# Aleph-Alpha/magma

Measured on NVIDIA H100. Metric: image-caption samples/sec (fwd+bwd), higher is better.
Workload: dtype bf16

## Files before the change

### include/magma_b200.h

```cpp
#ifndef MAGMA_B200_H_
#define MAGMA_B200_H_

#include <stddef.h>
#include <stdint.h>

#ifdef __cplusplus
extern "C" {
#endif

#define MB200_VERSION 100

enum {
  MB200_OK = 0,
  MB200_E_SHAPE = -1,
  MB200_E_DTYPE = -2,
  MB200_E_ALIGN = -3,
  MB200_E_ARCH = -4,
  MB200_E_CUDA = -5,
  MB200_E_NCCL = -6,
  MB200_E_ARG = -7
};

enum { MB200_BF16 = 0, MB200_F32 = 1 };

// ... 15 lines not shown
int mb200_check_device(void);
int mb200_set_gemm_sm_limit(int n_sms);
int mb200_set_optimizer_grid(int n_blocks);
long long mb200_launch_count(void);
int mb200_prof_enable(int on);
int mb200_prof_read(double* gemm_ms, double* gemm_flops, double* gemm_bytes, long long* gemm_launches);

typedef struct {
  const void* ptr;
  int64_t ld;
  int64_t bs0, bs1;
  int32_t mn_major;
  int32_t static_data;
} mb200_operand;

typedef struct {
  int32_t M, N, K;
  int32_t nb0, nb1;
  int32_t c_dtype;
  mb200_operand A, B;
  void* C;
  int64_t ldc, c_bs0, c_bs1;
  float alpha;
  int32_t act;
  int32_t dact;
  int32_t accumulate;
  const void* bias;
  void* aux_out;
  const void* aux_in;
  const void* res1;
  const void* res2;
  int64_t ld_res;
  int32_t force_bn;
  int32_t rope_mode;
  const void* rope_tab;
  int32_t rope_S, rope_hd, rope_rot, rope_ncols;
  void* splitk_ws;
  int64_t splitk_ws_bytes;
} mb200_gemm_args;

int mb200_gemm(const mb200_gemm_args* args, void* stream);


int mb200_layernorm_fwd(const void* x, int64_t ldx, const void* gamma, const void* beta, void* y, int64_t ldy,
                        float* mean, float* rstd, int32_t rows, int32_t d, float eps, void* stream);
int mb200_layernorm_bwd(const void* dy, int64_t lddy, const void* x, int64_t ldx, const void* gamma,
                        const float* mean, const float* rstd, const void* res, int64_t ldres, void* dx, int64_t lddx,
                        int32_t rows, int32_t d, void* stream);
int mb200_layernorm_param_grad(const void* dy, int64_t lddy, const void* x, int64_t ldx, const float* mean,
                               const float* rstd, float* dgamma, float* dbeta, int32_t rows, int32_t d,
                               int32_t accumulate, void* stream);
int mb200_layernorm_param_grad_rows(const void* dy, int64_t lddy, const void* x, int64_t ldx, const float* mean,
                                    const float* rstd, float* dgamma, float* dbeta, int32_t rows, int32_t d,
                                    int32_t accumulate, void* stream);
int mb200_rope(void* qkv, int64_t ld, int32_t rows, int32_t S, int32_t H, int32_t hd, int32_t rot, int32_t pos0,
               int32_t inverse, void* stream);
int mb200_rope_table(float* tab, int32_t S, int32_t rot, int32_t pos0, void* stream);
int mb200_softmax_fwd(const float* s, int64_t lds, int64_t s_bs, void* p, int64_t ldp, int64_t p_bs, int32_t nz,
                      int32_t Sq, int32_t Sk, float scale, int32_t causal, int32_t koff, void* stream);
int mb200_softmax_bwd(const float* dp, int64_t lddp, int64_t dp_bs, const void* p, int64_t ldp, int64_t p_bs,
                      void* ds, int64_t ldds, int64_t ds_bs, int32_t nz, int32_t Sq, int32_t Sk, float scale,
                      void* stream);
int mb200_build_labels(const int64_t* captions, int64_t ldc, int64_t* labels, int32_t B, int32_t S, int32_t L,
                       int64_t eos, void* stream);
int mb200_embed_assemble(const int64_t* captions, int64_t ldc, const void* wte, const void* prefix, int32_t L,
                         void* x, int32_t B, int32_t S, int32_t d, int32_t vocab, void* stream);
// ... 201 lines not shown
```

### magma_b200/_lib.py

```python
import ctypes
import os

_HERE = os.path.dirname(os.path.abspath(__file__))
LIB_PATH = os.path.join(_HERE, "lib", "libmagma_b200.so")

_lib = None


class MB200Error(RuntimeError):
    pass


class Operand(ctypes.Structure):
    _fields_ = [
        ("ptr", ctypes.c_void_p),
        ("ld", ctypes.c_int64),
        ("bs0", ctypes.c_int64),
        ("bs1", ctypes.c_int64),
        ("mn_major", ctypes.c_int32),
        ("static_data", ctypes.c_int32),
    ]


class GemmArgs(ctypes.Structure):
    _fields_ = [
        ("M", ctypes.c_int32),
        ("N", ctypes.c_int32),
        ("K", ctypes.c_int32),
        ("nb0", ctypes.c_int32),
        ("nb1", ctypes.c_int32),
        ("c_dtype", ctypes.c_int32),
        ("A", Operand),
        ("B", Operand),
        ("C", ctypes.c_void_p),
        ("ldc", ctypes.c_int64),
        ("c_bs0", ctypes.c_int64),
        ("c_bs1", ctypes.c_int64),
        ("alpha", ctypes.c_float),
        ("act", ctypes.c_int32),
        ("dact", ctypes.c_int32),
        ("accumulate", ctypes.c_int32),
        ("bias", ctypes.c_void_p),
        ("aux_out", ctypes.c_void_p),
        ("aux_in", ctypes.c_void_p),
        ("res1", ctypes.c_void_p),
        ("res2", ctypes.c_void_p),
        ("ld_res", ctypes.c_int64),
        ("force_bn", ctypes.c_int32),
        ("rope_mode", ctypes.c_int32),
        ("rope_tab", ctypes.c_void_p),
        ("rope_S", ctypes.c_int32),
        ("rope_hd", ctypes.c_int32),
        ("rope_rot", ctypes.c_int32),
        ("rope_ncols", ctypes.c_int32),
        ("splitk_ws", ctypes.c_void_p),
        ("splitk_ws_bytes", ctypes.c_int64),
    ]


def lib():
    global _lib
    if _lib is None:
        if not os.path.exists(LIB_PATH):
            raise MB200Error(
                f"{LIB_PATH} not found: build it with `python -m magma_b200.build` "
                "(magma_b200 has no CPU / eager fallback)"
            )
        L = ctypes.CDLL(LIB_PATH)
        L.mb200_last_error.restype = ctypes.c_char_p
        L.mb200_version.restype = ctypes.c_int
        _setup_signatures(L)
        _lib = L
    return _lib


def check(rc):
    if rc != 0:
        raise MB200Error(f"magma_b200 error {rc}: {lib().mb200_last_error().decode()}")


class VitLayerC(ctypes.Structure):
# ... 105 lines not shown
```

### magma_b200/csrc/gemm.cu

```cuda
#include <mutex>
#include <stdlib.h>

#include "gemm_common.cuh"

namespace mb200 {

template <bool kOn>
struct EpiMaps {
  CUtensorMap m[3];
};
template <>
struct EpiMaps<false> {};

template <int BN, bool A_MN, bool B_MN, bool EPI_TMA>
__global__ void __launch_bounds__(kThreads, 1)
gemm_wgmma_kernel(const __grid_constant__ CUtensorMap tmA, const __grid_constant__ CUtensorMap tmB,
                  const __grid_constant__ EpiMaps<EPI_TMA> tmE, const __grid_constant__ GemmKernelParams p) {
  using C_ = Cfg<BN>;
  constexpr int kStages = C_::kStages;

  extern __shared__ uint8_t smem_raw[];
  uint8_t* smem = reinterpret_cast<uint8_t*>((reinterpret_cast<uintptr_t>(smem_raw) + 1023) & ~uintptr_t(1023));
  uint8_t* smem_a = smem;
  uint8_t* smem_b = smem + kStages * C_::kABytes;
  float* epi_stage = reinterpret_cast<float*>(smem + kStages * C_::kStageBytes);
  uint64_t* full_bar = reinterpret_cast<uint64_t*>(smem + kStages * C_::kStageBytes + kEpiBytes);
  uint64_t* empty_bar = full_bar + kStages;
  const EpiRing ring{smem_a, smem_b, full_bar, empty_bar};

  const int wg = threadIdx.x >> 7;
  const int num_kb = (p.K + BK - 1) / BK;
  const int items = p.total_tiles * p.split_k;

  pdl_trigger();
  if (threadIdx.x == 0) {
    tma_prefetch_desc(&tmA);
    tma_prefetch_desc(&tmB);
    if constexpr (EPI_TMA) {
#pragma unroll 1
      for (int i = 0; i < p.epi_in; ++i) tma_prefetch_desc(&tmE.m[i]);
    }
    for (int s = 0; s < kStages; ++s) {
      mbar_init(&full_bar[s], 1);
      mbar_init(&empty_bar[s], 2);
    }
    mbar_fence_init();
  }
  __syncthreads();
  pdl_wait();

  if (wg == 0) {
    setmaxnreg_dec<40>();
    if (threadIdx.x == 0) {
      int stage = 0;
      uint32_t phase = 0;
// ... 47 lines not shown
    for (int w = blockIdx.x; w < items; w += gridDim.x) {
      const int t = w / p.split_k, ks = w - t * p.split_k;
      const int kb0 = ks * p.kb_per_split, kb1 = min(num_kb, kb0 + p.kb_per_split);
      const int tpb = p.tiles_m * p.tiles_n;
      const int z = t / tpb;
      const int r = t - z * tpb;
      const int m_blk = r % p.tiles_m;
      const int n_blk = r / p.tiles_m;
      const int z0 = z % p.nb0, z1 = z / p.nb0;
      int prev = -1;
      for (int kb = kb0; kb < kb1; ++kb) {
        mbar_wait(&full_bar[stage], phase);
        const uint32_t sa = smem_u32(smem_a + stage * C_::kABytes) + a_off;
        const uint32_t sb = smem_u32(smem_b + stage * C_::kBBytes);
        wgmma_fence();
#pragma unroll
        for (int k = 0; k < BK / WG_K; ++k) {
          const uint64_t da = make_smem_desc(sa + k * a_kadv, 0u, 1024);
          const uint64_t db = make_smem_desc(sb + k * b_kadv, b_lbo, 1024);
          wgmma_bf16<BN, A_MN ? 1 : 0, B_MN ? 1 : 0>(acc, da, db, (kb > kb0 || k > 0) ? 1u : 0u);
        }
        wgmma_commit();
        wgmma_wait<1>();
        if (prev >= 0 && leader) mbar_arrive(&empty_bar[prev]);
        prev = stage;
        if (++stage == kStages) {
          stage = 0;
          phase ^= 1;
        }
      }
      wgmma_wait<0>();
      if (prev >= 0 && leader) mbar_arrive(&empty_bar[prev]);
      const long long boff = (long long)z0 * p.c_bs0 + (long long)z1 * p.c_bs1;
      epi_tile<BN, EPI_TMA>(p, acc, epi_stage + cw * 64 * kEpiCols, 1 + cw, boff, m_blk * BM + cw * 64, n_blk * BN, ks, ring,
                   stage, phase);
    }
  }
}

__global__ void splitk_finalize_kernel(const GemmKernelParams p) {
  pdl_trigger();
  pdl_wait();
  const int ncol4 = (p.N + 3) >> 2;
  const long long total = (long long)p.M * ncol4;
  for (long long i = blockIdx.x * (long long)blockDim.x + threadIdx.x; i < total; i += (long long)gridDim.x * blockDim.x) {
    const int row = (int)(i / ncol4);
    const int col = (int)(i - (long long)row * ncol4) * 4;
    float v[4] = {0.f, 0.f, 0.f, 0.f};
    for (int ks = 0; ks < p.split_k; ++ks) {
      const float4 w4 = *reinterpret_cast<const float4*>(p.splitk_ws + ((long long)ks * p.M + row) * p.ld_ws + col);
      v[0] += w4.x;
      v[1] += w4.y;
      v[2] += w4.z;
      v[3] += w4.w;
    }
    EpiIn in;
    if (p.bias) ld_bf16x4(p.bias + col, min(4, p.N - col), in.bias);
    epi_load_inputs(p, 0, row, col, in);
    epi_store4(p, 0, row, col, v, in);
  }
}

typedef CUresult (*PFN_encodeTiled)(CUtensorMap*, CUtensorMapDataType, cuuint32_t, void*, const cuuint64_t*,
                                    const cuuint64_t*, const cuuint32_t*, const cuuint32_t*, CUtensorMapInterleave,
                                    CUtensorMapSwizzle, CUtensorMapL2promotion, CUtensorMapFloatOOBfill);

static PFN_encodeTiled get_encode_fn() {
  static PFN_encodeTiled fn = nullptr;
  static std::once_flag once;
  std::call_once(once, [] {
    void* p = nullptr;
    cudaDriverEntryPointQueryResult qres;
    if (cudaGetDriverEntryPoint("cuTensorMapEncodeTiled", &p, cudaEnableDefault, &qres) == cudaSuccess &&
        qres == cudaDriverEntryPointSuccess)
      fn = reinterpret_cast<PFN_encodeTiled>(p);
  });
  return fn;
}

int make_operand_map(CUtensorMap* out, const mb200_operand& op, int rows, int K, int nb0, int nb1,
                            int box_rows) {
  PFN_encodeTiled enc = get_encode_fn();
  MB_REQUIRE(enc != nullptr, MB200_E_CUDA, "cuTensorMapEncodeTiled entry point unavailable");
  MB_REQUIRE((reinterpret_cast<uintptr_t>(op.ptr) & 15) == 0, MB200_E_ALIGN, "gemm operand pointer not 16B aligned");
  MB_REQUIRE(op.ld % 8 == 0, MB200_E_ALIGN, "gemm operand ld (%lld) must be a multiple of 8 elements",
             (long long)op.ld);
  MB_REQUIRE((nb0 == 1 || op.bs0 % 8 == 0) && (nb1 == 1 || op.bs1 % 8 == 0), MB200_E_ALIGN,
             "gemm operand batch strides must be multiples of 8 elements");
  cuuint64_t dims[4];
  cuuint64_t strides[3];
  cuuint32_t box[4];
  cuuint32_t estr[4] = {1, 1, 1, 1};
  if (!op.mn_major) {
    dims[0] = (cuuint64_t)K;
    dims[1] = (cuuint64_t)rows;
    box[0] = BK;
    box[1] = (cuuint32_t)box_rows;
  } else {
    dims[0] = (cuuint64_t)rows;
    dims[1] = (cuuint64_t)K;
    box[0] = 64;
    box[1] = BK;
  }
  dims[2] = (cuuint64_t)nb0;
  dims[3] = (cuuint64_t)nb1;
  box[2] = 1;
  box[3] = 1;
  strides[0] = (cuuint64_t)op.ld * 2;
  strides[1] = (cuuint64_t)(nb0 > 1 ? op.bs0 : op.ld) * 2;
  strides[2] = (cuuint64_t)(nb1 > 1 ? op.bs1 : op.ld) * 2;
  CUresult r = enc(out, CU_TENSOR_MAP_DATA_TYPE_BFLOAT16, 4, const_cast<void*>(op.ptr), dims, strides, box, estr,
                   CU_TENSOR_MAP_INTERLEAVE_NONE, CU_TENSOR_MAP_SWIZZLE_128B, CU_TENSOR_MAP_L2_PROMOTION_L2_256B,
                   CU_TENSOR_MAP_FLOAT_OOB_FILL_NONE);
  MB_REQUIRE(r == CUDA_SUCCESS, MB200_E_CUDA,
             "cuTensorMapEncodeTiled failed (%d): dims=(%llu,%llu,%llu,%llu) strides=(%llu,%llu,%llu) box=(%u,%u)",
             (int)r, (unsigned long long)dims[0], (unsigned long long)dims[1], (unsigned long long)dims[2],
             (unsigned long long)dims[3], (unsigned long long)strides[0], (unsigned long long)strides[1],
             (unsigned long long)strides[2], box[0], box[1]);
  return 0;
}

template <int BN, bool A_MN, bool B_MN, bool EPI_TMA>
static int launch_gemm(const CUtensorMap& tmA, const CUtensorMap& tmB, const EpiMaps<true>& tmE,
                       const GemmKernelParams& kp, cudaStream_t stream) {
  auto kern = gemm_wgmma_kernel<BN, A_MN, B_MN, EPI_TMA>;
  static bool attr_set = false;
  if (!attr_set) {
    MB_CUDA(cudaFuncSetAttribute(kern, cudaFuncAttributeMaxDynamicSharedMemorySize, Cfg<BN>::kSmemBytes));
    attr_set = true;
  }
  const long long items = (long long)kp.total_tiles * kp.split_k;
  int grid = items < gemm_sms() ? (int)items : gemm_sms();
  {
    const double nb = (double)kp.total_tiles / ((double)kp.tiles_m * kp.tiles_n);
    const double flops = 2.0 * kp.M * (double)kp.N * kp.K * nb;
    const double bytes = nb * (2.0 * ((double)kp.M * kp.K + (double)kp.N * kp.K) + (kp.c_f32 ? 4.0 : 2.0) * kp.M * kp.N);
    GemmProfScope prof(stream, flops, bytes);
    if constexpr (EPI_TMA)
      MB_CUDA(launch_pdl(kern, dim3(grid), dim3(kThreads), Cfg<BN>::kSmemBytes, stream, tmA, tmB, tmE, kp));
    else
      MB_CUDA(launch_pdl(kern, dim3(grid), dim3(kThreads), Cfg<BN>::kSmemBytes, stream, tmA, tmB, EpiMaps<false>{}, kp));
  }
  count_launch();
  MB_CUDA(cudaGetLastError());
  return 0;
}

template <int BN, bool EPI_TMA>
static int dispatch_major(bool a_mn, bool b_mn, const CUtensorMap& tmA, const CUtensorMap& tmB,
                          const EpiMaps<true>& tmE, const GemmKernelParams& kp, cudaStream_t s) {
  if (!a_mn && !b_mn) return launch_gemm<BN, false, false, EPI_TMA>(tmA, tmB, tmE, kp, s);
  if (!a_mn && b_mn) return launch_gemm<BN, false, true, EPI_TMA>(tmA, tmB, tmE, kp, s);
  if (a_mn && !b_mn) return launch_gemm<BN, true, false, EPI_TMA>(tmA, tmB, tmE, kp, s);
  return launch_gemm<BN, true, true, EPI_TMA>(tmA, tmB, tmE, kp, s);
}

static int dispatch_bn(int bn, bool a_mn, bool b_mn, const CUtensorMap& tmA, const CUtensorMap& tmB,
                       const EpiMaps<true>& tmE, const GemmKernelParams& kp, cudaStream_t s) {
  const bool epi = kp.epi_in != 0;
  switch (bn) {
    case 64:
      return epi ? dispatch_major<64, true>(a_mn, b_mn, tmA, tmB, tmE, kp, s)
                 : dispatch_major<64, false>(a_mn, b_mn, tmA, tmB, tmE, kp, s);
    case 128:
      return epi ? dispatch_major<128, true>(a_mn, b_mn, tmA, tmB, tmE, kp, s)
                 : dispatch_major<128, false>(a_mn, b_mn, tmA, tmB, tmE, kp, s);
    default:
      return epi ? dispatch_major<256, true>(a_mn, b_mn, tmA, tmB, tmE, kp, s)
                 : dispatch_major<256, false>(a_mn, b_mn, tmA, tmB, tmE, kp, s);
  }
}

static int make_epi_maps(EpiMaps<true>* maps, GemmKernelParams* kp, const mb200_gemm_args* a) {
  const void* ptr[3];
  long long ld[3];
  int n = 0;
  if (a->dact) {
    ptr[n] = a->aux_in;
    ld[n++] = a->ldc;
  }
  if (a->res1) {
    ptr[n] = a->res1;
    ld[n++] = a->ld_res;
  }
  if (a->res2) {
    ptr[n] = a->res2;
    ld[n++] = a->ld_res;
  }
  bool ok = (a->nb0 == 1 || a->c_bs0 % 8 == 0) && (a->nb1 == 1 || a->c_bs1 % 8 == 0);
  for (int i = 0; i < n; ++i) ok = ok && (reinterpret_cast<uintptr_t>(ptr[i]) & 15) == 0 && ld[i] % 8 == 0;
  if (n == 0 || !ok) return 0;
  for (int i = 0; i < n; ++i) {
    mb200_operand op;
    memset(&op, 0, sizeof(op));
    op.ptr = ptr[i];
    op.ld = ld[i];
    op.bs0 = a->c_bs0;
    op.bs1 = a->c_bs1;
    const int rc = make_operand_map(&maps->m[i], op, a->M, a->N, a->nb0, a->nb1, BM);
    if (rc) return rc;
  }
  kp->epi_in = n;
  return 0;
// ... 145 lines not shown
    }
    const long long ld_ws = (a->N + 3) / 4 * 4;
    while (split > 1 && (size_t)split * a->M * ld_ws * sizeof(float) > (size_t)a->splitk_ws_bytes) --split;
    if (split > 1) {
      const int kb_per = (num_kb + split - 1) / split;
      split = (num_kb + kb_per - 1) / kb_per;
      bn = bn_s;
      rc = make_operand_map(&tmB, a->B, a->N, a->K, a->nb0, a->nb1, bn);
      if (rc) return rc;
      kp.tiles_n = tiles;
      kp.total_tiles = tiles_m * tiles;
      kp.split_k = split;
      kp.kb_per_split = kb_per;
      kp.splitk_ws = reinterpret_cast<float*>(a->splitk_ws);
      kp.ld_ws = ld_ws;
      GemmKernelParams kg = kp;
      kg.epi_kind = EK_SPLITK;
      rc = dispatch_bn(bn, amn, bmn, tmA, tmB, tmE, kg, stream);
      if (rc) return rc;
      const long long n4 = (long long)a->M * ((a->N + 3) / 4);
      const int fgrid = (int)((n4 + 255) / 256 > 2048 ? 2048 : (n4 + 255) / 256);
      kp.alpha = 1.f;
      MB_CUDA(launch_pdl(splitk_finalize_kernel, dim3(fgrid), dim3(256), 0, stream, kp));
      count_launch();
      return 0;
    }
  }
  rc = make_operand_map(&tmB, a->B, a->N, a->K, a->nb0, a->nb1, bn);
  if (rc) return rc;
  kp.tiles_n = (a->N + bn - 1) / bn;
  kp.total_tiles = tiles_m * kp.tiles_n * a->nb0 * a->nb1;
  rc = make_epi_maps(&tmE, &kp, a);
  if (rc) return rc;
  return dispatch_bn(bn, amn, bmn, tmA, tmB, tmE, kp, stream);
}

}

extern "C" int mb200_gemm(const mb200_gemm_args* args, void* stream) {
  return mb200::gemm_impl(args, reinterpret_cast<cudaStream_t>(stream));
}
```

### magma_b200/csrc/gemm_common.cuh

```cuda
#pragma once
#include "common.cuh"

namespace mb200 {

static constexpr int BM = 128;
static constexpr int BK = 64;
static constexpr int WG_K = 16;
static constexpr int kThreads = 384;
static constexpr int kEpiCols = 64;
static constexpr int kEpiBytes = BM * kEpiCols * 4;
static constexpr int kEpiBoxBytes = BM * kEpiCols * 2;
static constexpr int kSmemBudget = 192 * 1024;

template <int BN>
struct Cfg {
  static constexpr int kABytes = BM * BK * 2;
  static constexpr int kBBytes = BN * BK * 2;
  static constexpr int kStageBytes = kABytes + kBBytes;
  static constexpr int kStagesRaw = kSmemBudget / kStageBytes;
  static constexpr int kStages = kStagesRaw > 8 ? 8 : kStagesRaw;
  static constexpr int kSmemBytes = kStages * kStageBytes + kEpiBytes + 1024  + 256 ;
  static_assert(kSmemBytes <= 227 * 1024, "GEMM shared memory exceeds the sm_90 per-block limit");
  static constexpr int kEpiBoxesPerStage = 1 + kBBytes / kEpiBoxBytes;
  static_assert(kABytes == kEpiBoxBytes && kEpiBoxesPerStage * kEpiBoxBytes <= kStageBytes, "epilogue box layout");
  static_assert(3 * (BN / kEpiCols) <= kStages * kEpiBoxesPerStage, "epilogue inputs exceed the operand ring");
};

struct GemmKernelParams {
  int M, N, K;
  int nb0;
  int tiles_m, tiles_n, total_tiles;
  void* C;
  long long ldc, c_bs0, c_bs1;
  float alpha;
  int act, dact, accumulate;
  const bf16* bias;
  bf16* aux_out;
  const bf16* aux_in;
  const bf16* res1;
  const bf16* res2;
  long long ld_res;
  int epi_in;
  const float2* rope_tab;
  int rope_mode;
  int rope_S, rope_hd, rope_rot, rope_ncols;
  int epi_kind;
  int c_f32;
  int split_k, kb_per_split;
  float* splitk_ws;
  long long ld_ws;
};

__device__ __forceinline__ float2 bf16x2_to_f32(uint32_t u) {
  return __bfloat1622float2(*reinterpret_cast<const __nv_bfloat162*>(&u));
}
__device__ __forceinline__ uint32_t f32x2_to_bf16(float a, float b) {
  __nv_bfloat162 h = __floats2bfloat162_rn(a, b);
  return *reinterpret_cast<uint32_t*>(&h);
}

__device__ __forceinline__ void ld_bf16x4(const bf16* src, int n, float (&v)[4]) {
  if (n == 4 && (reinterpret_cast<uintptr_t>(src) & 7) == 0) {
    uint32_t u0, u1;
    asm volatile("ld.global.nc.v2.u32 {%0, %1}, [%2];" : "=r"(u0), "=r"(u1) : "l"(src));
    const float2 a = bf16x2_to_f32(u0), b = bf16x2_to_f32(u1);
    v[0] = a.x;
    v[1] = a.y;
    v[2] = b.x;
    v[3] = b.y;
  } else {
#pragma unroll
    for (int e = 0; e < 4; ++e) v[e] = e < n ? __bfloat162float(src[e]) : 0.f;
  }
}
__device__ __forceinline__ void st_bf16x4(bf16* dst, int n, const float (&v)[4]) {
  if (n == 4 && (reinterpret_cast<uintptr_t>(dst) & 7) == 0) {
    *reinterpret_cast<uint2*>(dst) = make_uint2(f32x2_to_bf16(v[0], v[1]), f32x2_to_bf16(v[2], v[3]));
  } else {
#pragma unroll
    for (int e = 0; e < 4; ++e)
      if (e < n) dst[e] = __float2bfloat16(v[e]);
  }
}

__device__ __forceinline__ void named_bar_sync(int id, int nthreads) {
  asm volatile("bar.sync %0, %1;" ::"r"(id), "r"(nthreads) : "memory");
}

enum { EK_GENERIC = 0, EK_SPLITK };

struct EpiIn {
  float bias[4], aux[4], res1[4], res2[4];
};

__device__ __forceinline__ void epi_load_inputs(const GemmKernelParams& p, long long boff, int row, int col,
                                                EpiIn& in) {
  const int n = min(4, p.N - col);
  if (p.dact) ld_bf16x4(p.aux_in + boff + (long long)row * p.ldc + col, n, in.aux);
  const long long roff = boff + (long long)row * p.ld_res + col;
  if (p.res1) ld_bf16x4(p.res1 + roff, n, in.res1);
  if (p.res2) ld_bf16x4(p.res2 + roff, n, in.res2);
}

__device__ __forceinline__ void ld_smem_bf16x4(const uint8_t* src, float (&v)[4]) {
  const uint2 u = *reinterpret_cast<const uint2*>(src);
  const float2 a = bf16x2_to_f32(u.x), b = bf16x2_to_f32(u.y);
  v[0] = a.x;
  v[1] = a.y;
  v[2] = b.x;
  v[3] = b.y;
}

__device__ __forceinline__ void epi_store4(const GemmKernelParams& p, long long boff, int row, int col, float (&v)[4],
                                           const EpiIn& in) {
  const int n = min(4, p.N - col);
  if (p.bias) {
#pragma unroll
    for (int e = 0; e < 4; ++e) v[e] += in.bias[e];
  }
  if (p.rope_mode != 0 && col < p.rope_ncols) {
    const int dim = col % p.rope_hd;
    if (dim < p.rope_rot) {
      const float2* tp = p.rope_tab + (long long)(row % p.rope_S) * (p.rope_rot >> 1) + (dim >> 1);
      const float2 cs0 = __ldg(tp), cs1 = __ldg(tp + 1);
      const float sg = p.rope_mode > 0 ? 1.f : -1.f;
      const float a0 = v[0], a1 = v[1], a2 = v[2], a3 = v[3];
      v[0] = a0 * cs0.x - a1 * cs0.y * sg;
      v[1] = a1 * cs0.x + a0 * cs0.y * sg;
      v[2] = a2 * cs1.x - a3 * cs1.y * sg;
      v[3] = a3 * cs1.x + a2 * cs1.y * sg;
    }
  }
  const long long coff = boff + (long long)row * p.ldc + col;
  if (p.aux_out) st_bf16x4(p.aux_out + coff, n, v);
#pragma unroll
  for (int e = 0; e < 4; ++e) {
    if (p.act == MB200_ACT_GELU_NEW) v[e] = gelu_new_f(v[e]);
    else if (p.act == MB200_ACT_QUICK_GELU) v[e] = quick_gelu_f(v[e]);
    else if (p.act == MB200_ACT_RELU) v[e] = fmaxf(v[e], 0.f);
  }
  if (p.dact) {
#pragma unroll
    for (int e = 0; e < 4; ++e)
      v[e] = p.dact == MB200_DACT_GELU_NEW ? v[e] * gelu_new_grad_f(in.aux[e]) : (in.aux[e] > 0.f ? v[e] : 0.f);
  }
  if (p.res1) {
#pragma unroll
    for (int e = 0; e < 4; ++e) v[e] += in.res1[e];
  }
  if (p.res2) {
#pragma unroll
    for (int e = 0; e < 4; ++e) v[e] += in.res2[e];
  }
  if (p.act == MB200_ACT_RELU_POST) {
#pragma unroll
    for (int e = 0; e < 4; ++e) v[e] = fmaxf(v[e], 0.f);
  }
  if (p.c_f32) {
    float* dst = reinterpret_cast<float*>(p.C) + coff;
    if (n == 4) {
      float4 o = make_float4(v[0], v[1], v[2], v[3]);
      if (p.accumulate) {
        const float4 old = *reinterpret_cast<const float4*>(dst);
        o.x += old.x;
        o.y += old.y;
        o.z += old.z;
        o.w += old.w;
      }
      *reinterpret_cast<float4*>(dst) = o;
    } else {
#pragma unroll
      for (int e = 0; e < 4; ++e)
        if (e < n) dst[e] = p.accumulate ? dst[e] + v[e] : v[e];
    }
  } else {
    st_bf16x4(reinterpret_cast<bf16*>(p.C) + coff, n, v);
  }
}


struct EpiRing {
  uint8_t* a;
  uint8_t* b;
  uint64_t* full;
  uint64_t* empty;
};

template <int BN>
__device__ __forceinline__ int epi_chunks(const GemmKernelParams& p, int col0) {
  return min(BN / kEpiCols, (p.N - col0 + kEpiCols - 1) / kEpiCols);
}

template <int BN>
__device__ __forceinline__ uint8_t* epi_box(const EpiRing& ring, int s, int k) {
  return k == 0 ? ring.a + s * Cfg<BN>::kABytes : ring.b + s * Cfg<BN>::kBBytes + (k - 1) * kEpiBoxBytes;
}

template <int BN, bool EPI_TMA>
__device__ __forceinline__ void epi_tile(const GemmKernelParams& p, const float (&acc)[BN / 2], float* stage,
                                         int bar_id, long long boff, int row0, int col0, int ks, const EpiRing& ring,
                                         int& ring_stage, uint32_t& ring_phase) {
  constexpr int kStages = Cfg<BN>::kStages, kBps = Cfg<BN>::kEpiBoxesPerStage;
  const int wt = threadIdx.x & 127;
  const int fr = (wt >> 5) * 16 + ((wt & 31) >> 2);
  const int fq = wt & 3;
  const int pr = wt >> 4, pc = wt & 15;
  const int nch = epi_chunks<BN>(p, col0);
  const int nin = EPI_TMA ? p.epi_in : 0;
  int bs = ring_stage, bk = 0, rs = ring_stage;
  uint32_t bph = ring_phase;
  auto next_box = [&]() {
    if (bk == 0) mbar_wait(&ring.full[bs], bph);
    const uint8_t* box = epi_box<BN>(ring, bs, bk);
    if (++bk == kBps) {
      bk = 0;
      if (++bs == kStages) {
        bs = 0;
        bph ^= 1;
      }
    }
    return box;
  };
  const int box_off = ((row0 % BM) + pr) * 128 + (((pc >> 1) ^ pr) << 4) + ((pc & 1) << 3);
#pragma unroll 1
  for (int ch = 0; ch < nch; ++ch) {
#pragma unroll
    for (int c = 0; c < BN / kEpiCols; ++c) {
      if (c != ch) continue;
#pragma unroll
      for (int jj = 0; jj < 8; ++jj) {
        const int j = c * 8 + jj;
#pragma unroll
        for (int h = 0; h < 2; ++h) {
          const int r = fr + 8 * h;
          const int q = (2 * jj + (fq >> 1)) ^ ((r & 3) << 1);
          *reinterpret_cast<float2*>(stage + r * kEpiCols + q * 4 + 2 * (fq & 1)) =
              make_float2(acc[4 * j + 2 * h], acc[4 * j + 2 * h + 1]);
        }
      }
    }
    named_bar_sync(bar_id, 128);
    const int col = col0 + ch * kEpiCols + pc * 4;
    const uint8_t *src_aux = nullptr, *src_res1 = nullptr, *src_res2 = nullptr;
    if (nin) {
      if (p.dact) src_aux = next_box() + box_off;
      if (p.res1) src_res1 = next_box() + box_off;
      if (p.res2) src_res2 = next_box() + box_off;
    }
    EpiIn in;
    if (p.bias && col < p.N) ld_bf16x4(p.bias + col, min(4, p.N - col), in.bias);
#pragma unroll 1
    for (int i = 0; i < 64 / 8; ++i) {
      const int r = pr + 8 * i;
      const int row = row0 + r;
      if (row >= p.M || col >= p.N) continue;
      const float4 s = *reinterpret_cast<const float4*>(stage + r * kEpiCols + ((pc ^ ((r & 3) << 1)) * 4));
      float v[4] = {s.x * p.alpha, s.y * p.alpha, s.z * p.alpha, s.w * p.alpha};
      if (p.epi_kind == EK_SPLITK) {
        *reinterpret_cast<float4*>(p.splitk_ws + ((long long)ks * p.M + row) * p.ld_ws + col) =
            make_float4(v[0], v[1], v[2], v[3]);
        continue;
      }
      if (nin) {
        if (p.dact) ld_smem_bf16x4(src_aux + i * 1024, in.aux);
        if (p.res1) ld_smem_bf16x4(src_res1 + i * 1024, in.res1);
        if (p.res2) ld_smem_bf16x4(src_res2 + i * 1024, in.res2);
      } else {
        epi_load_inputs(p, boff, row, col, in);
      }
      epi_store4(p, boff, row, col, v, in);
    }
    named_bar_sync(bar_id, 128);
    if (nin) {
      if (ch + 1 == nch && bk != 0) {
        bk = 0;
        if (++bs == kStages) {
          bs = 0;
          bph ^= 1;
        }
      }
#pragma unroll 1
      for (; rs != bs; rs = rs + 1 == kStages ? 0 : rs + 1)
        if (wt == 0) mbar_arrive(&ring.empty[rs]);
    }
  }
  ring_stage = bs;
  ring_phase = bph;
}

template <int BN>
__device__ __forceinline__ void epi_queue_inputs(const GemmKernelParams& p, const CUtensorMap* maps,
                                                 const EpiRing& ring, int& stage, uint32_t& phase, int m0, int col0,
                                                 int z0, int z1) {
  constexpr int kStages = Cfg<BN>::kStages, kBps = Cfg<BN>::kEpiBoxesPerStage;
  const int nbox = p.epi_in * epi_chunks<BN>(p, col0);
  int col = col0, i = 0;
#pragma unroll 1
  for (int b0 = 0; b0 < nbox; b0 += kBps) {
    const int nb = min(kBps, nbox - b0);
    mbar_wait(&ring.empty[stage], phase ^ 1);
    mbar_expect_tx(&ring.full[stage], (uint32_t)(nb * kEpiBoxBytes));
#pragma unroll 1
    for (int k = 0; k < nb; ++k) {
// ... 17 lines not shown
```

### magma_b200/ops.py

```python
import ctypes

import torch

from . import _lib
from ._lib import GemmArgs, check, lib

ACT_NONE, ACT_GELU_NEW, ACT_QUICK_GELU, ACT_RELU, ACT_RELU_POST = 0, 1, 2, 3, 4
DACT_NONE, DACT_GELU_NEW, DACT_RELU = 0, 1, 3


def _stream():
    return ctypes.c_void_p(torch.cuda.current_stream().cuda_stream)


def _ptr(t):
    return ctypes.c_void_p(t.data_ptr()) if t is not None else None


def _mat_meta(t, name):
    if t.dim() < 2 or t.dim() > 4:
        raise ValueError(f"{name}: expected 2-4 dims, got {t.dim()}")
    if t.stride(-1) != 1 and t.shape[-1] != 1:
        raise ValueError(f"{name}: innermost stride must be 1, got {t.stride()}")
    rows, cols = t.shape[-2], t.shape[-1]
    ld = t.stride(-2) if rows > 1 else max(cols, t.stride(-2))
    nb0 = t.shape[-3] if t.dim() >= 3 else 1
    bs0 = t.stride(-3) if t.dim() >= 3 else 0
    nb1 = t.shape[-4] if t.dim() >= 4 else 1
    bs1 = t.stride(-4) if t.dim() >= 4 else 0
    return rows, cols, ld, nb0, nb1, bs0, bs1


def gemm(
    A,
    B,
    out=None,
    *,
    a_mn=False,
    b_mn=False,
    out_dtype=torch.bfloat16,
    alpha=1.0,
    bias=None,
    act=ACT_NONE,
    aux_out=None,
    aux_in=None,
    dact=DACT_NONE,
    res1=None,
    res2=None,
    accumulate=False,
    force_bn=0,
    rope_tab=None,
    rope_mode=0,
    rope_S=0,
    rope_hd=0,
    rope_rot=0,
    rope_ncols=0,
    splitk_ws=None,
    b_static=False,
):
    if A.dtype != torch.bfloat16 or B.dtype != torch.bfloat16:
        raise TypeError("gemm operands must be bf16")
    ra, ca, lda, anb0, anb1, abs0, abs1 = _mat_meta(A, "A")
    rb, cb, ldb, bnb0, bnb1, bbs0, bbs1 = _mat_meta(B, "B")
    M, K = (ca, ra) if a_mn else (ra, ca)
    N, Kb = (cb, rb) if b_mn else (rb, cb)
    if K != Kb:
        raise ValueError(f"gemm K mismatch: {K} vs {Kb}")
    nb0, nb1 = max(anb0, bnb0), max(anb1, bnb1)
    if (anb0, anb1) != (nb0, nb1) or (bnb0, bnb1) != (nb0, nb1):
        raise ValueError("gemm: A and B must have identical batch dims")
    if out is None:
        shape = ([nb1] if A.dim() >= 4 else []) + ([nb0] if A.dim() >= 3 else []) + [M, N]
        out = torch.empty(shape, dtype=out_dtype, device=A.device)
    rc_, cc, ldc, cnb0, cnb1, cbs0, cbs1 = _mat_meta(out, "out")
    if (rc_, cc) != (M, N) or (cnb0, cnb1) != (nb0, nb1):
        raise ValueError(f"gemm: out shape {tuple(out.shape)} does not match M={M} N={N} batch=({nb1},{nb0})")
    g = GemmArgs()
    g.M, g.N, g.K, g.nb0, g.nb1 = M, N, K, nb0, nb1
    g.c_dtype = 1 if out.dtype == torch.float32 else 0
    if out.dtype not in (torch.float32, torch.bfloat16):
        raise TypeError("gemm out must be bf16 or f32")
    g.A.ptr, g.A.ld, g.A.bs0, g.A.bs1, g.A.mn_major = A.data_ptr(), lda, abs0, abs1, int(a_mn)
    g.B.ptr, g.B.ld, g.B.bs0, g.B.bs1, g.B.mn_major = B.data_ptr(), ldb, bbs0, bbs1, int(b_mn)
    g.B.static_data = int(bool(b_static))
    g.C, g.ldc, g.c_bs0, g.c_bs1 = out.data_ptr(), ldc, cbs0, cbs1
    g.alpha, g.act, g.dact, g.accumulate = float(alpha), int(act), int(dact), int(bool(accumulate))
    for name, t in (("bias", bias), ("aux_out", aux_out), ("aux_in", aux_in), ("res1", res1), ("res2", res2)):
        if t is not None:
            if t.dtype != torch.bfloat16:
                raise TypeError(f"gemm {name} must be bf16")
            setattr(g, name, t.data_ptr())
    if bias is not None and (tuple(bias.shape) != (N,) or (N > 1 and bias.stride(0) != 1)):
        raise ValueError(f"gemm bias must be a contiguous [N={N}] vector, got shape {tuple(bias.shape)}")
    for name, t in (("aux_out", aux_out), ("aux_in", aux_in), ("res1", res1), ("res2", res2)):
        if t is not None and tuple(t.shape) != tuple(out.shape):
            raise ValueError(f"gemm {name} shape {tuple(t.shape)} must equal out's {tuple(out.shape)}")
    for name, t in (("aux_out", aux_out), ("aux_in", aux_in)):
        if t is not None and _mat_meta(t, name)[2:] != (ldc, cnb0, cnb1, cbs0, cbs1):
            raise ValueError(f"gemm {name} must share out's strides")
    ld_res = 0
    for name, t in (("res1", res1), ("res2", res2)):
        if t is not None:
            m = _mat_meta(t, name)
            if (cnb0 > 1 and m[5] != cbs0) or (cnb1 > 1 and m[6] != cbs1):
                raise ValueError(f"gemm {name} must share out's batch strides (its row stride may differ)")
            if ld_res and m[2] != ld_res:
                raise ValueError("res1/res2 must share a row stride")
            ld_res = m[2]
    g.ld_res = ld_res
    g.force_bn = force_bn
    if rope_tab is not None and rope_mode:
        g.rope_tab, g.rope_mode = rope_tab.data_ptr(), int(rope_mode)
        g.rope_S, g.rope_hd, g.rope_rot, g.rope_ncols = int(rope_S), int(rope_hd), int(rope_rot), int(rope_ncols)
    if splitk_ws is not None:
        g.splitk_ws, g.splitk_ws_bytes = splitk_ws.data_ptr(), splitk_ws.numel() * splitk_ws.element_size()
    check(lib().mb200_gemm(ctypes.byref(g), _stream()))
    return out


def _rows(t):
    d = t.shape[-1]
    if t.dim() == 1:
        return 1, d, d
    t2 = t.reshape(-1, d) if t.is_contiguous() else None
    if t2 is not None:
        return t2.shape[0], d, d
    if t.dim() == 2:
        return t.shape[0], d, t.stride(0)
    raise ValueError("non-contiguous >2-D tensor: pass a 2-D view with an explicit row stride")


def layernorm_fwd(x, gamma, beta, eps=1e-5, save_stats=True, out=None):
    rows, d, ldx = _rows(x)
    y = torch.empty(x.shape, dtype=torch.bfloat16, device=x.device) if out is None else out
    mean = torch.empty(rows, dtype=torch.float32, device=x.device) if save_stats else None
    rstd = torch.empty(rows, dtype=torch.float32, device=x.device) if save_stats else None
    check(lib().mb200_layernorm_fwd(_ptr(x), ctypes.c_int64(ldx), _ptr(gamma), _ptr(beta), _ptr(y),
                                    ctypes.c_int64(_rows(y)[2]), _ptr(mean), _ptr(rstd), rows, d,
                                    ctypes.c_float(eps), _stream()))
    return y, mean, rstd


def layernorm_bwd(dy, x, gamma, mean, rstd, res=None, out=None):
# ... 413 lines not shown
```

Measured before the change: 136.7.

## Specialize GEMM epilogue at compile time for common fusion forms

Adds compile-time epilogue variants (EpiForm) for a set of common fused-epilogue combinations: bias, GELU, aux output, residuals, dGELU, RoPE and f32 output. A host-side dispatcher picks the matching specialized kernel when BN is 256 and the alignment checks pass. Specialized forms drop runtime branches, process 8 rows per unrolled batch and use unconditional vector loads and stores. This is meant to cut epilogue instruction overhead and raise memory-level parallelism, at the cost of more kernel instantiations, longer compile time and higher register pressure.

After: 155.5 (median of 6 runs). 13.7% higher.

```diff
diff --git a/include/magma_b200.h b/include/magma_b200.h
--- a/include/magma_b200.h
+++ b/include/magma_b200.h
@@ -71,6 +71,7 @@
   const void* res2;
   int64_t ld_res;
   int32_t force_bn;
+  int32_t generic_epilogue;
   int32_t rope_mode;
   const void* rope_tab;
   int32_t rope_S, rope_hd, rope_rot, rope_ncols;
diff --git a/magma_b200/_lib.py b/magma_b200/_lib.py
--- a/magma_b200/_lib.py
+++ b/magma_b200/_lib.py
@@ -47,6 +47,7 @@
         ("res2", ctypes.c_void_p),
         ("ld_res", ctypes.c_int64),
         ("force_bn", ctypes.c_int32),
+        ("generic_epilogue", ctypes.c_int32),
         ("rope_mode", ctypes.c_int32),
         ("rope_tab", ctypes.c_void_p),
         ("rope_S", ctypes.c_int32),
diff --git a/magma_b200/csrc/gemm.cu b/magma_b200/csrc/gemm.cu
--- a/magma_b200/csrc/gemm.cu
+++ b/magma_b200/csrc/gemm.cu
@@ -12,7 +12,7 @@
 template <>
 struct EpiMaps<false> {};
 
-template <int BN, bool A_MN, bool B_MN, bool EPI_TMA>
+template <int BN, bool A_MN, bool B_MN, bool EPI_TMA, uint32_t FORM = EF_RUNTIME>
 __global__ void __launch_bounds__(kThreads, 1)
 gemm_wgmma_kernel(const __grid_constant__ CUtensorMap tmA, const __grid_constant__ CUtensorMap tmB,
                   const __grid_constant__ EpiMaps<EPI_TMA> tmE, const __grid_constant__ GemmKernelParams p) {
@@ -20,7 +20,7 @@
   constexpr int kStages = C_::kStages;
 
   extern __shared__ uint8_t smem_raw[];
-  uint8_t* smem = reinterpret_cast<uint8_t*>((reinterpret_cast<uintptr_t>(smem_raw) + 1023) & ~uintptr_t(1023));
+  uint8_t* smem = smem_raw + ((1024u - (smem_u32(smem_raw) & 1023u)) & 1023u);
   uint8_t* smem_a = smem;
   uint8_t* smem_b = smem + kStages * C_::kABytes;
   float* epi_stage = reinterpret_cast<float*>(smem + kStages * C_::kStageBytes);
@@ -134,8 +134,8 @@
       wgmma_wait<0>();
       if (prev >= 0 && leader) mbar_arrive(&empty_bar[prev]);
       const long long boff = (long long)z0 * p.c_bs0 + (long long)z1 * p.c_bs1;
-      epi_tile<BN, EPI_TMA>(p, acc, epi_stage + cw * 64 * kEpiCols, 1 + cw, boff, m_blk * BM + cw * 64, n_blk * BN, ks, ring,
-                   stage, phase);
+      epi_tile<BN, EPI_TMA, EpiForm<FORM>>(p, acc, epi_stage + cw * 64 * kEpiCols, 1 + cw, boff, m_blk * BM + cw * 64,
+                                           n_blk * BN, ks, ring, stage, phase);
     }
   }
 }
@@ -156,10 +156,12 @@
       v[2] += w4.z;
       v[3] += w4.w;
     }
+    using Form = EpiForm<EF_RUNTIME>;
+    float bias[4];
     EpiIn in;
-    if (p.bias) ld_bf16x4(p.bias + col, min(4, p.N - col), in.bias);
-    epi_load_inputs(p, 0, row, col, in);
-    epi_store4(p, 0, row, col, v, in);
+    if (p.bias) ld_bf16x4(p.bias + col, min(4, p.N - col), bias);
+    epi_load_inputs<Form>(p, 0, row, col, in);
+    epi_store4<Form>(p, 0, row, col, v, bias, in);
   }
 }
 
@@ -222,10 +224,10 @@
   return 0;
 }
 
-template <int BN, bool A_MN, bool B_MN, bool EPI_TMA>
+template <int BN, bool A_MN, bool B_MN, bool EPI_TMA, uint32_t FORM = EF_RUNTIME>
 static int launch_gemm(const CUtensorMap& tmA, const CUtensorMap& tmB, const EpiMaps<true>& tmE,
                        const GemmKernelParams& kp, cudaStream_t stream) {
-  auto kern = gemm_wgmma_kernel<BN, A_MN, B_MN, EPI_TMA>;
+  auto kern = gemm_wgmma_kernel<BN, A_MN, B_MN, EPI_TMA, FORM>;
   static bool attr_set = false;
   if (!attr_set) {
     MB_CUDA(cudaFuncSetAttribute(kern, cudaFuncAttributeMaxDynamicSharedMemorySize, Cfg<BN>::kSmemBytes));
@@ -271,6 +273,41 @@
       return epi ? dispatch_major<256, true>(a_mn, b_mn, tmA, tmB, tmE, kp, s)
                  : dispatch_major<256, false>(a_mn, b_mn, tmA, tmB, tmE, kp, s);
   }
+}
+
+template <uint32_t F, bool A_MN, bool B_MN>
+static bool launch_form(uint32_t form, bool a_mn, bool b_mn, const CUtensorMap& tmA, const CUtensorMap& tmB,
+                        const EpiMaps<true>& tmE, const GemmKernelParams& kp, cudaStream_t s, int* rc) {
+  if (form != F || a_mn != A_MN || b_mn != B_MN) return false;
+  *rc = launch_gemm<256, A_MN, B_MN, EpiForm<F>::kInputs != 0, F>(tmA, tmB, tmE, kp, s);
+  return true;
+}
+static bool dispatch_form(uint32_t form, bool a_mn, bool b_mn, const CUtensorMap& tmA, const CUtensorMap& tmB,
+                          const EpiMaps<true>& tmE, const GemmKernelParams& kp, cudaStream_t s, int* rc) {
+#define MB_FORM(F, A_MN, B_MN) launch_form<(F), A_MN, B_MN>(form, a_mn, b_mn, tmA, tmB, tmE, kp, s, rc)
+  return MB_FORM(EF_ROPE, false, false) ||
+         MB_FORM(EF_RES1, false, false) ||
+         MB_FORM(EF_BIAS | EF_GELU | EF_AUX_OUT, false, false) ||
+         MB_FORM(EF_BIAS, false, false) ||
+         MB_FORM(EF_BIAS | EF_RES1 | EF_RES2, false, false) ||
+         MB_FORM(EF_DGELU, false, true) ||
+         MB_FORM(0u, false, true) ||
+         MB_FORM(EF_RES1, false, true) ||
+         MB_FORM(EF_F32, true, true);
+#undef MB_FORM
+}
+
+static uint32_t epi_form(const mb200_gemm_args* a, const GemmKernelParams& kp, int bn) {
+  if (a->generic_epilogue || bn != 256) return EF_RUNTIME;
+  if ((a->act != MB200_ACT_NONE && a->act != MB200_ACT_GELU_NEW) ||
+      (a->dact != MB200_DACT_NONE && a->dact != MB200_DACT_GELU_NEW))
+    return EF_RUNTIME;
+  if (((reinterpret_cast<uintptr_t>(a->bias) | reinterpret_cast<uintptr_t>(a->aux_out)) & 7) != 0) return EF_RUNTIME;
+  const uint32_t f = (a->bias ? EF_BIAS : 0u) | (kp.rope_mode ? EF_ROPE : 0u) | (a->aux_out ? EF_AUX_OUT : 0u) |
+                     (a->act ? EF_GELU : 0u) | (a->dact ? EF_DGELU : 0u) | (a->res1 ? EF_RES1 : 0u) |
+                     (a->res2 ? EF_RES2 : 0u) | (kp.c_f32 ? EF_F32 : 0u);
+  const int inputs = (a->dact != 0) + (a->res1 != nullptr) + (a->res2 != nullptr);
+  return kp.epi_in == inputs ? f : EF_RUNTIME;
 }
 
 static int make_epi_maps(EpiMaps<true>* maps, GemmKernelParams* kp, const mb200_gemm_args* a) {
@@ -482,6 +519,7 @@
   kp.total_tiles = tiles_m * kp.tiles_n * a->nb0 * a->nb1;
   rc = make_epi_maps(&tmE, &kp, a);
   if (rc) return rc;
+  if (dispatch_form(epi_form(a, kp, bn), amn, bmn, tmA, tmB, tmE, kp, stream, &rc)) return rc;
   return dispatch_bn(bn, amn, bmn, tmA, tmB, tmE, kp, stream);
 }
 
diff --git a/magma_b200/csrc/gemm_common.cuh b/magma_b200/csrc/gemm_common.cuh
--- a/magma_b200/csrc/gemm_common.cuh
+++ b/magma_b200/csrc/gemm_common.cuh
@@ -1,4 +1,6 @@
 #pragma once
+#include <type_traits>
+
 #include "common.cuh"
 
 namespace mb200 {
@@ -59,8 +61,9 @@
   return *reinterpret_cast<uint32_t*>(&h);
 }
 
+template <bool kVec = false>
 __device__ __forceinline__ void ld_bf16x4(const bf16* src, int n, float (&v)[4]) {
-  if (n == 4 && (reinterpret_cast<uintptr_t>(src) & 7) == 0) {
+  if (kVec || (n == 4 && (reinterpret_cast<uintptr_t>(src) & 7) == 0)) {
     uint32_t u0, u1;
     asm volatile("ld.global.nc.v2.u32 {%0, %1}, [%2];" : "=r"(u0), "=r"(u1) : "l"(src));
     const float2 a = bf16x2_to_f32(u0), b = bf16x2_to_f32(u1);
@@ -73,8 +76,9 @@
     for (int e = 0; e < 4; ++e) v[e] = e < n ? __bfloat162float(src[e]) : 0.f;
   }
 }
+template <bool kVec = false>
 __device__ __forceinline__ void st_bf16x4(bf16* dst, int n, const float (&v)[4]) {
-  if (n == 4 && (reinterpret_cast<uintptr_t>(dst) & 7) == 0) {
+  if (kVec || (n == 4 && (reinterpret_cast<uintptr_t>(dst) & 7) == 0)) {
     *reinterpret_cast<uint2*>(dst) = make_uint2(f32x2_to_bf16(v[0], v[1]), f32x2_to_bf16(v[2], v[3]));
   } else {
 #pragma unroll
@@ -89,17 +93,54 @@
 
 enum { EK_GENERIC = 0, EK_SPLITK };
 
+enum : uint32_t {
+  EF_BIAS = 1,
+  EF_ROPE = 2,
+  EF_AUX_OUT = 4,
+  EF_GELU = 8,
+  EF_DGELU = 16,
+  EF_RES1 = 32,
+  EF_RES2 = 64,
+  EF_F32 = 128,
+  EF_RUNTIME = 1u << 31
+};
+
+template <uint32_t F>
+struct EpiForm {
+  static constexpr bool kRuntime = F == EF_RUNTIME;
+  static constexpr int kInputs = kRuntime ? 0 : ((F & EF_DGELU) != 0) + ((F & EF_RES1) != 0) + ((F & EF_RES2) != 0);
+  static constexpr int kRows = kRuntime ? 1 : 8;
+  using P = GemmKernelParams;
+  static __device__ __forceinline__ bool bias(const P& p) { return kRuntime ? p.bias != nullptr : (F & EF_BIAS) != 0; }
+  static __device__ __forceinline__ bool rope(const P& p) { return kRuntime ? p.rope_mode != 0 : (F & EF_ROPE) != 0; }
+  static __device__ __forceinline__ bool aux_out(const P& p) {
+    return kRuntime ? p.aux_out != nullptr : (F & EF_AUX_OUT) != 0;
+  }
+  static __device__ __forceinline__ int act(const P& p) {
+    return kRuntime ? p.act : (F & EF_GELU) ? MB200_ACT_GELU_NEW : MB200_ACT_NONE;
+  }
+  static __device__ __forceinline__ int dact(const P& p) {
+    return kRuntime ? p.dact : (F & EF_DGELU) ? MB200_DACT_GELU_NEW : MB200_DACT_NONE;
+  }
+  static __device__ __forceinline__ bool res1(const P& p) { return kRuntime ? p.res1 != nullptr : (F & EF_RES1) != 0; }
+  static __device__ __forceinline__ bool res2(const P& p) { return kRuntime ? p.res2 != nullptr : (F & EF_RES2) != 0; }
+  static __device__ __forceinline__ bool c_f32(const P& p) { return kRuntime ? p.c_f32 != 0 : (F & EF_F32) != 0; }
+  static __device__ __forceinline__ bool accumulate(const P& p) { return (kRuntime || (F & EF_F32)) && p.accumulate; }
+  static __device__ __forceinline__ bool splitk(const P& p) { return kRuntime && p.epi_kind == EK_SPLITK; }
+};
+
 struct EpiIn {
-  float bias[4], aux[4], res1[4], res2[4];
-};
-
+  float aux[4], res1[4], res2[4];
+};
+
+template <class Form>
 __device__ __forceinline__ void epi_load_inputs(const GemmKernelParams& p, long long boff, int row, int col,
                                                 EpiIn& in) {
   const int n = min(4, p.N - col);
-  if (p.dact) ld_bf16x4(p.aux_in + boff + (long long)row * p.ldc + col, n, in.aux);
+  if (Form::dact(p)) ld_bf16x4(p.aux_in + boff + (long long)row * p.ldc + col, n, in.aux);
   const long long roff = boff + (long long)row * p.ld_res + col;
-  if (p.res1) ld_bf16x4(p.res1 + roff, n, in.res1);
-  if (p.res2) ld_bf16x4(p.res2 + roff, n, in.res2);
+  if (Form::res1(p)) ld_bf16x4(p.res1 + roff, n, in.res1);
+  if (Form::res2(p)) ld_bf16x4(p.res2 + roff, n, in.res2);
 }
 
 __device__ __forceinline__ void ld_smem_bf16x4(const uint8_t* src, float (&v)[4]) {
@@ -111,14 +152,15 @@
   v[3] = b.y;
 }
 
+template <class Form, bool kVec = false>
 __device__ __forceinline__ void epi_store4(const GemmKernelParams& p, long long boff, int row, int col, float (&v)[4],
-                                           const EpiIn& in) {
+                                           const float (&bias)[4], const EpiIn& in) {
   const int n = min(4, p.N - col);
-  if (p.bias) {
-#pragma unroll
-    for (int e = 0; e < 4; ++e) v[e] += in.bias[e];
-  }
-  if (p.rope_mode != 0 && col < p.rope_ncols) {
+  if (Form::bias(p)) {
+#pragma unroll
+    for (int e = 0; e < 4; ++e) v[e] += bias[e];
+  }
+  if (Form::rope(p) && col < p.rope_ncols) {
     const int dim = col % p.rope_hd;
     if (dim < p.rope_rot) {
       const float2* tp = p.rope_tab + (long long)(row % p.rope_S) * (p.rope_rot >> 1) + (dim >> 1);
@@ -132,35 +174,35 @@
     }
   }
   const long long coff = boff + (long long)row * p.ldc + col;
-  if (p.aux_out) st_bf16x4(p.aux_out + coff, n, v);
+  if (Form::aux_out(p)) st_bf16x4<kVec>(p.aux_out + coff, n, v);
 #pragma unroll
   for (int e = 0; e < 4; ++e) {
-    if (p.act == MB200_ACT_GELU_NEW) v[e] = gelu_new_f(v[e]);
-    else if (p.act == MB200_ACT_QUICK_GELU) v[e] = quick_gelu_f(v[e]);
-    else if (p.act == MB200_ACT_RELU) v[e] = fmaxf(v[e], 0.f);
-  }
-  if (p.dact) {
+    if (Form::act(p) == MB200_ACT_GELU_NEW) v[e] = gelu_new_f(v[e]);
+    else if (Form::act(p) == MB200_ACT_QUICK_GELU) v[e] = quick_gelu_f(v[e]);
+    else if (Form::act(p) == MB200_ACT_RELU) v[e] = fmaxf(v[e], 0.f);
+  }
+  if (Form::dact(p)) {
 #pragma unroll
     for (int e = 0; e < 4; ++e)
-      v[e] = p.dact == MB200_DACT_GELU_NEW ? v[e] * gelu_new_grad_f(in.aux[e]) : (in.aux[e] > 0.f ? v[e] : 0.f);
-  }
-  if (p.res1) {
+      v[e] = Form::dact(p) == MB200_DACT_GELU_NEW ? v[e] * gelu_new_grad_f(in.aux[e]) : (in.aux[e] > 0.f ? v[e] : 0.f);
+  }
+  if (Form::res1(p)) {
 #pragma unroll
     for (int e = 0; e < 4; ++e) v[e] += in.res1[e];
   }
-  if (p.res2) {
+  if (Form::res2(p)) {
 #pragma unroll
     for (int e = 0; e < 4; ++e) v[e] += in.res2[e];
   }
-  if (p.act == MB200_ACT_RELU_POST) {
+  if (Form::act(p) == MB200_ACT_RELU_POST) {
 #pragma unroll
     for (int e = 0; e < 4; ++e) v[e] = fmaxf(v[e], 0.f);
   }
-  if (p.c_f32) {
+  if (Form::c_f32(p)) {
     float* dst = reinterpret_cast<float*>(p.C) + coff;
-    if (n == 4) {
+    if (kVec || n == 4) {
       float4 o = make_float4(v[0], v[1], v[2], v[3]);
-      if (p.accumulate) {
+      if (Form::accumulate(p)) {
         const float4 old = *reinterpret_cast<const float4*>(dst);
         o.x += old.x;
         o.y += old.y;
@@ -171,10 +213,10 @@
     } else {
 #pragma unroll
       for (int e = 0; e < 4; ++e)
-        if (e < n) dst[e] = p.accumulate ? dst[e] + v[e] : v[e];
+        if (e < n) dst[e] = Form::accumulate(p) ? dst[e] + v[e] : v[e];
     }
   } else {
-    st_bf16x4(reinterpret_cast<bf16*>(p.C) + coff, n, v);
+    st_bf16x4<kVec>(reinterpret_cast<bf16*>(p.C) + coff, n, v);
   }
 }
 
@@ -196,7 +238,7 @@
   return k == 0 ? ring.a + s * Cfg<BN>::kABytes : ring.b + s * Cfg<BN>::kBBytes + (k - 1) * kEpiBoxBytes;
 }
 
-template <int BN, bool EPI_TMA>
+template <int BN, bool EPI_TMA, class Form>
 __device__ __forceinline__ void epi_tile(const GemmKernelParams& p, const float (&acc)[BN / 2], float* stage,
                                          int bar_id, long long boff, int row0, int col0, int ks, const EpiRing& ring,
                                          int& ring_stage, uint32_t& ring_phase) {
@@ -206,7 +248,7 @@
   const int fq = wt & 3;
   const int pr = wt >> 4, pc = wt & 15;
   const int nch = epi_chunks<BN>(p, col0);
-  const int nin = EPI_TMA ? p.epi_in : 0;
+  const int nin = !EPI_TMA ? 0 : Form::kRuntime ? p.epi_in : Form::kInputs;
   int bs = ring_stage, bk = 0, rs = ring_stage;
   uint32_t bph = ring_phase;
   auto next_box = [&]() {
@@ -243,32 +285,52 @@
     const int col = col0 + ch * kEpiCols + pc * 4;
     const uint8_t *src_aux = nullptr, *src_res1 = nullptr, *src_res2 = nullptr;
     if (nin) {
-      if (p.dact) src_aux = next_box() + box_off;
-      if (p.res1) src_res1 = next_box() + box_off;
-      if (p.res2) src_res2 = next_box() + box_off;
-    }
-    EpiIn in;
-    if (p.bias && col < p.N) ld_bf16x4(p.bias + col, min(4, p.N - col), in.bias);
-#pragma unroll 1
-    for (int i = 0; i < 64 / 8; ++i) {
-      const int r = pr + 8 * i;
-      const int row = row0 + r;
-      if (row >= p.M || col >= p.N) continue;
-      const float4 s = *reinterpret_cast<const float4*>(stage + r * kEpiCols + ((pc ^ ((r & 3) << 1)) * 4));
-      float v[4] = {s.x * p.alpha, s.y * p.alpha, s.z * p.alpha, s.w * p.alpha};
-      if (p.epi_kind == EK_SPLITK) {
-        *reinterpret_cast<float4*>(p.splitk_ws + ((long long)ks * p.M + row) * p.ld_ws + col) =
-            make_float4(v[0], v[1], v[2], v[3]);
-        continue;
-      }
-      if (nin) {
-        if (p.dact) ld_smem_bf16x4(src_aux + i * 1024, in.aux);
-        if (p.res1) ld_smem_bf16x4(src_res1 + i * 1024, in.res1);
-        if (p.res2) ld_smem_bf16x4(src_res2 + i * 1024, in.res2);
+      if (Form::dact(p)) src_aux = next_box() + box_off;
+      if (Form::res1(p)) src_res1 = next_box() + box_off;
+      if (Form::res2(p)) src_res2 = next_box() + box_off;
+    }
+    const int n = min(4, p.N - col);
+    float bias[4];
+    if (Form::bias(p) && col < p.N) ld_bf16x4(p.bias + col, n, bias);
+    auto rows = [&](auto rows_c, auto vec_c, int i0) {
+      constexpr int kRows = decltype(rows_c)::value;
+      constexpr bool kVec = decltype(vec_c)::value;
+      float4 s[kRows];
+      EpiIn in[kRows];
+#pragma unroll
+      for (int u = 0; u < kRows; ++u) {
+        const int i = i0 + u, r = pr + 8 * i;
+        s[u] = *reinterpret_cast<const float4*>(stage + r * kEpiCols + ((pc ^ ((r & 3) << 1)) * 4));
+        if (nin) {
+          if (Form::dact(p)) ld_smem_bf16x4(src_aux + i * 1024, in[u].aux);
+          if (Form::res1(p)) ld_smem_bf16x4(src_res1 + i * 1024, in[u].res1);
+          if (Form::res2(p)) ld_smem_bf16x4(src_res2 + i * 1024, in[u].res2);
+        }
+      }
+#pragma unroll
+      for (int u = 0; u < kRows; ++u) {
+        const int row = row0 + pr + 8 * (i0 + u);
+        if (row >= p.M) continue;
+        float v[4] = {__fmul_rn(s[u].x, p.alpha), __fmul_rn(s[u].y, p.alpha), __fmul_rn(s[u].z, p.alpha),
+                      __fmul_rn(s[u].w, p.alpha)};
+        if (Form::splitk(p)) {
+          *reinterpret_cast<float4*>(p.splitk_ws + ((long long)ks * p.M + row) * p.ld_ws + col) =
+              make_float4(v[0], v[1], v[2], v[3]);
+          continue;
+        }
+        if (!nin) epi_load_inputs<Form>(p, boff, row, col, in[u]);
+        epi_store4<Form, kVec>(p, boff, row, col, v, bias, in[u]);
+      }
+    };
+    if (col < p.N) {
+      if (Form::kRuntime || n == 4) {
+#pragma unroll 1
+        for (int i0 = 0; i0 < 64 / 8; i0 += Form::kRows)
+          rows(std::integral_constant<int, Form::kRows>(), std::integral_constant<bool, !Form::kRuntime>(), i0);
       } else {
-        epi_load_inputs(p, boff, row, col, in);
-      }
-      epi_store4(p, boff, row, col, v, in);
+#pragma unroll 1
+        for (int i0 = 0; i0 < 64 / 8; ++i0) rows(std::integral_constant<int, 1>(), std::false_type(), i0);
+      }
     }
     named_bar_sync(bar_id, 128);
     if (nin) {
diff --git a/magma_b200/ops.py b/magma_b200/ops.py
--- a/magma_b200/ops.py
+++ b/magma_b200/ops.py
@@ -49,6 +49,7 @@
     res2=None,
     accumulate=False,
     force_bn=0,
+    generic_epilogue=False,
     rope_tab=None,
     rope_mode=0,
     rope_S=0,
@@ -109,6 +110,7 @@
             ld_res = m[2]
     g.ld_res = ld_res
     g.force_bn = force_bn
+    g.generic_epilogue = int(bool(generic_epilogue))
     if rope_tab is not None and rope_mode:
         g.rope_tab, g.rope_mode = rope_tab.data_ptr(), int(rope_mode)
         g.rope_S, g.rope_hd, g.rope_rot, g.rope_ncols = int(rope_S), int(rope_hd), int(rope_rot), int(rope_ncols)
```
